# hirofumi0810/tensorflow_end2end_speech_recognition

Measured on AMD Instinct MI355X. Metric: acoustic frames/sec (train), TIMIT-shaped BLSTM-CTC, higher is better.
Workload: dtype bf16; 1 GPU; TIMIT 61-phone 5x256 BLSTM-CTC, B=16/GPU, D=120, C=62, seq_len~U{100..778}, dropout 0.2, rmsprop, train step; global_batch=16, parallelism=dp1, padded_to=own Tmax per rank

## Files before the change

### include/asr_hip.h

```cpp
#ifndef ASR_HIP_H_
#define ASR_HIP_H_

#include <stddef.h>
#include <stdint.h>

#ifdef __cplusplus
extern "C" {
#endif

typedef struct asr_handle asr_handle;
typedef void* asr_stream;

typedef enum {
  ASR_OK = 0,
  ASR_ERR_INVALID_ARG = -1,
  ASR_ERR_UNSUPPORTED = -2,
  ASR_ERR_HIP = -3,
  ASR_ERR_WORKSPACE = -4
} asr_status;

typedef enum { ASR_F32 = 0, ASR_BF16 = 1 } asr_dtype;

typedef enum {
  ASR_OPT_SGD = 0, ASR_OPT_MOMENTUM = 1, ASR_OPT_NESTEROV = 2, ASR_OPT_ADAGRAD = 3,
// ... 17 lines not shown
int asr_stack_frames(asr_handle* h, const float* x, const int32_t* seq_len, int B, int T, int F,
                     int num_stack, int num_skip, float* out, int32_t* out_len, asr_stream s);
int asr_splice(asr_handle* h, const float* x, const int32_t* seq_len, int B, int T, int D, int splice,
               int num_stack, float* out, asr_stream s);
int asr_transpose2d(asr_handle* h, int dtype, const void* in, int rows, int cols, int ld_in,
                    void* out, int ld_out, asr_stream s);
int asr_cast_from_f32(asr_handle* h, int dtype, const float* in, void* out, size_t n, asr_stream s);
int asr_cast_to_f32(asr_handle* h, int dtype, const void* in, float* out, size_t n, asr_stream s);
int asr_apply_mask(asr_handle* h, int dtype, const void* in, const float* mask, void* out,
                   size_t n, asr_stream s);
int asr_touch(asr_handle* h, const void* p, size_t bytes, asr_stream s);
int asr_dropout_mask(asr_handle* h, float* mask, size_t n, float keep_prob,
                     uint64_t seed, uint64_t offset, asr_stream s);
int asr_dropout_apply(asr_handle* h, int dtype, const void* in, void* out, size_t n, float keep_prob, uint64_t seed,
                      uint64_t offset, asr_stream s);
int asr_relu_bwd_drop(asr_handle* h, int dtype, const float* dout, const void* out, size_t n, float keep_prob,
                      uint64_t seed, uint64_t offset, void* dpre, asr_stream s);
int asr_colsum(asr_handle* h, int dtype, const void* a, int M, int N, int lda,
               float* out, asr_stream s);

int asr_gemm(asr_handle* h, int dtype, int out_dtype, int transA, int transB,
             int M, int N, int K, const void* A, int lda, const void* B, int ldb,
             void* C, int ldc, const float* bias, int accumulate, asr_stream s);

int asr_gemm_act(asr_handle* h, int dtype, int out_dtype, int transA, int transB,
                 int M, int N, int K, const void* A, int lda, const void* B, int ldb,
                 void* C, int ldc, const float* bias, int accumulate, int act, asr_stream s);
int asr_gemm_mul(asr_handle* h, int dtype, int transA, int transB, int M, int N, int K,
                 const void* A, int lda, const void* B, int ldb, float* C, int ldc,
                 const float* bias, int accumulate, int act, const float* mul, int ldmul, asr_stream s);
int asr_gemm_drop(asr_handle* h, int dtype, int transA, int transB, int M, int N, int K, const void* A, int lda,
                  const void* B, int ldb, float* C, int ldc, const float* bias, int accumulate, int act, float keep_prob,
                  uint64_t seed, uint64_t offset, asr_stream s);

int asr_im2col3x3(asr_handle* h, int dtype, const void* in, int N, int H, int W, int Cin, int ldp,
                  void* patches, asr_stream s);
int asr_col2im3x3(asr_handle* h, const float* dpatches, int N, int H, int W, int Cin, int ldp,
                  float* din, asr_stream s);
int asr_im2col(asr_handle* h, int dtype, const void* in_nhwc, int N, int H, int W, int Cin, int kh, int kw,
               int sh, int sw, int ldp, void* patches, asr_stream s);
int asr_col2im(asr_handle* h, const float* dpatches, int N, int H, int W, int Cin, int kh, int kw,
               int sh, int sw, int ldp, float* din_nhwc, asr_stream s);
int asr_conv3x3_prep_weights(asr_handle* h, const float* w_hwio, int Cin, int Cout, void* wt_fwd,
                             void* wt_bwd, asr_stream s);
int asr_conv3x3_fwd(asr_handle* h, const void* x, int N, int H, int W, int Cin, const void* wt_fwd,
                    const float* bias, int Cout, int relu, void* out, asr_stream s);
int asr_conv3x3_fwd_drop(asr_handle* h, const void* x, int N, int H, int W, int Cin, const void* wt_fwd,
                         const float* bias, int Cout, float keep_prob, uint64_t seed, uint64_t offset, void* out,
                         asr_stream s);
int asr_conv3x3_bwd_data(asr_handle* h, const void* dy, int N, int H, int W, int Cout,
                         const void* wt_bwd, int Cin, float* dx, asr_stream s);
int asr_conv3x3_bwd_data_relu(asr_handle* h, const void* dy, int N, int H, int W, int Cout, const void* wt_bwd, int Cin,
                              const void* act_below, float keep_prob, uint64_t seed, uint64_t offset, int use_drop,
                              void* dpre_below, asr_stream s);
int asr_conv3x3_bwd_weight(asr_handle* h, const void* x, const void* dy, int N, int H, int W,
                           int Cin, int Cout, float* dw, int accumulate, asr_stream s);
int asr_conv3x3_bwd_weight_bias(asr_handle* h, const void* x, const void* dy, int N, int H, int W,
                                int Cin, int Cout, float* dw, float* dbias, asr_stream s);
int asr_maxpool2x2_fwd(asr_handle* h, int dtype, const void* in, int N, int H, int W, int C,
                       void* out, uint8_t* argmax, asr_stream s);
int asr_maxpool2x2_fwd_drop(asr_handle* h, int dtype, const void* in, int N, int H, int W, int C, void* out,
                            uint8_t* argmax, float keep_prob, uint64_t seed, uint64_t offset, asr_stream s);
int asr_maxpool2x2_bwd(asr_handle* h, const float* dout, const uint8_t* argmax, int N, int H, int W,
                       int C, float* din, asr_stream s);
int asr_conv3x3_smallc_fwd(asr_handle* h, const void* x, int N, int H, int W, int Cin, const void* w2d,
                           const float* bias, int Cout, int relu, void* out, asr_stream s);
// ... 235 lines not shown
```

### tensorflow_end2end_speech_recognition_amd/_lib.py

```python
import ctypes as C
import os

_PKG = os.path.dirname(os.path.abspath(__file__))
LIB_PATH = os.path.join(_PKG, 'libasr_hip.so')

ASR_F32, ASR_BF16 = 0, 1
OPTIMIZER_IDS = {'sgd': 0, 'momentum': 1, 'nestrov': 2, 'adagrad': 3, 'adadelta': 4,
                 'rmsprop': 5, 'adam': 6}

_vp, _i, _f, _sz = C.c_void_p, C.c_int, C.c_float, C.c_size_t
_i64, _u64 = C.c_int64, C.c_uint64

SIGNATURES = {
    'asr_abi_version': (_i, []),
    'asr_create': (_i, [C.POINTER(_vp), _i]),
    'asr_create_ex': (_i, [C.POINTER(_vp), _i, _sz]),
    'asr_scratch_bytes': (_sz, [_vp]),
    'asr_destroy': (_i, [_vp]),
    'asr_set_xcd_skip': (_i, [_vp, _i]),
    'asr_set_gemm_tn_workgroups': (_i, [_vp, _i]),
    'asr_last_error_string': (C.c_char_p, [_vp]),
    'asr_device_info': (_i, [_vp, C.POINTER(_i), C.c_char_p, _i]),
    'asr_bt_to_tb': (_i, [_vp, _i, _vp, _vp, _i, _i, _i, _vp]),
    'asr_bt_to_tb_ld': (_i, [_vp, _i, _vp, _vp, _i, _i, _i, _i, _vp]),
    'asr_transpose2d': (_i, [_vp, _i, _vp, _i, _i, _i, _vp, _i, _vp]),
    'asr_cast_from_f32': (_i, [_vp, _i, _vp, _vp, _sz, _vp]),
    'asr_cast_to_f32': (_i, [_vp, _i, _vp, _vp, _sz, _vp]),
    'asr_apply_mask': (_i, [_vp, _i, _vp, _vp, _vp, _sz, _vp]),
    'asr_dropout_mask': (_i, [_vp, _vp, _sz, _f, _u64, _u64, _vp]),
    'asr_touch': (_i, [_vp, _vp, _sz, _vp]),
    'asr_dropout_apply': (_i, [_vp, _i, _vp, _vp, _sz, _f, _u64, _u64, _vp]),
    'asr_relu_bwd_drop': (_i, [_vp, _i, _vp, _vp, _sz, _f, _u64, _u64, _vp, _vp]),
    'asr_colsum': (_i, [_vp, _i, _vp, _i, _i, _i, _vp, _vp]),
    'asr_gemm': (_i, [_vp, _i, _i, _i, _i, _i, _i, _i, _vp, _i, _vp, _i, _vp, _i, _vp, _i, _vp]),
    'asr_gemm_act': (_i, [_vp, _i, _i, _i, _i, _i, _i, _i, _vp, _i, _vp, _i, _vp, _i, _vp, _i, _i, _vp]),
    'asr_gemm_drop': (_i, [_vp, _i, _i, _i, _i, _i, _i, _vp, _i, _vp, _i, _vp, _i, _vp, _i, _i, _f, _u64, _u64, _vp]),
    'asr_gemm_mul': (_i, [_vp, _i, _i, _i, _i, _i, _i, _vp, _i, _vp, _i, _vp, _i, _vp, _i, _i, _vp, _i, _vp]),
    'asr_conv3x3_prep_weights': (_i, [_vp, _vp, _i, _i, _vp, _vp, _vp]),
    'asr_conv3x3_fwd': (_i, [_vp, _vp, _i, _i, _i, _i, _vp, _vp, _i, _i, _vp, _vp]),
    'asr_conv3x3_fwd_drop': (_i, [_vp, _vp, _i, _i, _i, _i, _vp, _vp, _i, _f, _u64, _u64, _vp, _vp]),
    'asr_conv3x3_bwd_data': (_i, [_vp, _vp, _i, _i, _i, _i, _vp, _i, _vp, _vp]),
    'asr_conv3x3_smallc_fwd': (_i, [_vp, _vp, _i, _i, _i, _i, _vp, _vp, _i, _i, _vp, _vp]),
    'asr_conv3x3_smallc_fwd_drop': (_i, [_vp, _vp, _i, _i, _i, _i, _vp, _vp, _i, _f, _u64, _u64, _vp, _vp]),
    'asr_conv3x3_smallc_bwd_weight': (_i, [_vp, _vp, _vp, _i, _i, _i, _i, _i, _vp, _vp]),
    'asr_conv3x3_smallc_bwd_weight_bias': (_i, [_vp, _vp, _vp, _i, _i, _i, _i, _i, _vp, _vp, _vp]),
    'asr_conv3x3_bwd_data_relu': (_i, [_vp, _vp, _i, _i, _i, _i, _vp, _i, _vp, _f, _u64, _u64, _i, _vp, _vp]),
    'asr_conv3x3_bwd_weight': (_i, [_vp, _vp, _vp, _i, _i, _i, _i, _i, _vp, _i, _vp]),
    'asr_conv3x3_bwd_weight_bias': (_i, [_vp, _vp, _vp, _i, _i, _i, _i, _i, _vp, _vp, _vp]),
    'asr_im2col3x3': (_i, [_vp, _i, _vp, _i, _i, _i, _i, _i, _vp, _vp]),
    'asr_col2im3x3': (_i, [_vp, _vp, _i, _i, _i, _i, _i, _vp, _vp]),
    'asr_im2col': (_i, [_vp, _i, _vp, _i, _i, _i, _i, _i, _i, _i, _i, _i, _vp, _vp]),
    'asr_col2im': (_i, [_vp, _vp, _i, _i, _i, _i, _i, _i, _i, _i, _i, _vp, _vp]),
    'asr_maxpool2x2_fwd': (_i, [_vp, _i, _vp, _i, _i, _i, _i, _vp, _vp, _vp]),
    'asr_maxpool2x2_fwd_drop': (_i, [_vp, _i, _vp, _i, _i, _i, _i, _vp, _vp, _f, _u64, _u64, _vp]),
    'asr_relu_bwd_scaled': (_i, [_vp, _i, _vp, _vp, _sz, _f, _vp, _vp]),
    'asr_maxpool2x2_bwd': (_i, [_vp, _vp, _vp, _i, _i, _i, _i, _vp, _vp]),
    'asr_relu_bwd': (_i, [_vp, _i, _vp, _vp, _vp, _sz, _vp, _vp]),
    'asr_maxpool2x2_relu_bwd': (_i, [_vp, _i, _vp, _vp, _vp, _i, _i, _i, _i, _vp, _f, _u64, _u64, _i, _vp]),
    'asr_conv3x5_prep_weights': (_i, [_vp, _vp, _i, _i, _vp, _vp, _vp]),
    'asr_conv3x5_fwd': (_i, [_vp, _vp, _i, _i, _i, _i, _vp, _vp, _i, _i, _vp, _vp]),
    'asr_conv3x5_fwd_drop': (_i, [_vp, _vp, _i, _i, _i, _i, _vp, _vp, _i, _f, _u64, _u64, _vp, _vp]),
    'asr_conv3x5_bwd_data': (_i, [_vp, _vp, _i, _i, _i, _i, _vp, _i, _vp, _vp]),
    'asr_conv3x5_bwd_data_relu': (_i, [_vp, _vp, _i, _i, _i, _i, _vp, _i, _vp, _f, _u64, _u64, _i, _vp, _vp]),
    'asr_conv3x5_bwd_weight_bias': (_i, [_vp, _vp, _vp, _i, _i, _i, _i, _i, _vp, _vp, _vp]),
    'asr_maxpool3x1_fwd': (_i, [_vp, _i, _vp, _i, _i, _i, _i, _vp, _vp, _f, _u64, _u64, _i, _vp]),
    'asr_maxpool3x1_bwd': (_i, [_vp, _i, _vp, _vp, _i, _i, _i, _i, _vp, _vp]),
    'asr_lstm_prep_weights': (_i, [_vp, _i, _vp, _vp, _i, _i, _vp, _vp, _vp, _vp, _vp]),
    'asr_lstm_prep_layer': (_i, [_vp, _i, _i, _vp, _i, _i, _i, _vp, _vp, _vp, _vp, _vp, _vp, _vp]),
    'asr_lstm_grad_finish': (_i, [_vp, _i, _vp, _i, _i, _vp, _vp, _i, _vp]),
    'asr_gate_deinterleave': (_i, [_vp, _vp, _i, _vp, _i, _i, _i, _vp]),
# ... 147 lines not shown
```

### tensorflow_end2end_speech_recognition_amd/csrc/gemm.hip

```cpp
#include "common.h"
#include <stdlib.h>

namespace {

static inline bool first_on_device(unsigned long long& mask) {
  int d = 0;
  (void)hipGetDevice(&d);
  const unsigned long long bit = 1ull << (d & 63);
  if (mask & bit) return false;
  mask |= bit;
  return true;
}

template <typename T> struct GT;
template <> struct GT<float> {
  static constexpr int BK = 32;
  static constexpr int VEC = 4;
};
template <> struct GT<bf16_t> {
  static constexpr int BK = 64;
  static constexpr int VEC = 8;
};

template <typename T> struct Vec16 { T v[GT<T>::VEC]; } __attribute__((aligned(16)));
// ... 178 lines not shown
          *reinterpret_cast<f32x4_t*>(cp) = (f32x4_t){v[0], v[1], v[2], v[3]};
        } else {
          typedef __attribute__((ext_vector_type(4))) unsigned short us4_t;
          if (accumulate) {
            const us4_t o = *reinterpret_cast<const us4_t*>(cp);
#pragma unroll
            for (int r = 0; r < 4; ++r) v[r] += bf16_to_f32(o[r]);
          }
          if (act == 1) {
#pragma unroll
            for (int r = 0; r < 4; ++r) v[r] = fmaxf(v[r], 0.f);
          }
          *reinterpret_cast<us4_t*>(cp) = (us4_t){f32_to_bf16(v[0]), f32_to_bf16(v[1]), f32_to_bf16(v[2]), f32_to_bf16(v[3])};
        }
      } else {
        for (int r = 0; r < 4 && nb + r < N; ++r) {
          float w = v[r];
          if (accumulate) w += load_out<TO>(cp + r);
          if (act == 1) w = fmaxf(w, 0.f);
          store_out<TO>(cp + r, w);
        }
      }
    }
}

__device__ __forceinline__ unsigned nt_swz(int row) { return (((row + 4) >> 3) & 1) ? 8u : 0u; }

struct GemmDrop {
  float keep;
  uint64_t seed, offset;
  int use;
};

template <typename TO>
__global__ __launch_bounds__(256) void gemm_nt_bf16_kernel(int M, int N, int K, const bf16_t* __restrict__ A,
                                                           int lda, const bf16_t* __restrict__ Bt, int ldb,
                                                           TO* __restrict__ C, int ldc,
                                                           const float* __restrict__ bias, int accumulate,
                                                           int act, const float* __restrict__ mul, int ldm,
                                                           GemmDrop drop) {
  constexpr int BM = 128, BN = 128, BK = 64, LD = BK + 8;
  constexpr int STAGE = (BM + BN) * LD;
  extern __shared__ __attribute__((aligned(16))) char smem[];
  bf16_t* S = reinterpret_cast<bf16_t*>(smem);

  const int tid = threadIdx.x, lane = tid & 63, wave = tid >> 6;
  const int wm = wave >> 1, wn = wave & 1;
  const int ntn = N / BN, ntm = (M + BM - 1) / BM, total = ntn * ntm;
  int t = blockIdx.x;
  if ((total & 7) == 0) t = (t & 7) * (total >> 3) + (t >> 3);
  const int m0 = (t / ntn) * BM, n0 = (t % ntn) * BN;

  const bf16_t* pa[4];
  const bf16_t* pb[4];
  unsigned so[4];
#pragma unroll
  for (int i = 0; i < 4; ++i) {
    const int v = tid + i * 256, r = v >> 3, kv = (v & 7) * 8;
    pa[i] = A + (size_t)min(m0 + r, M - 1) * lda + kv;
    pb[i] = Bt + (size_t)(n0 + r) * ldb + kv;
    so[i] = (unsigned)(r * LD) + ((unsigned)kv ^ nt_swz(r));
  }
  bf16x8_t ra[4], rb[4];
  auto gload = [&]() {
#pragma unroll
    for (int i = 0; i < 4; ++i) {
      ra[i] = *reinterpret_cast<const bf16x8_t*>(pa[i]);
      rb[i] = *reinterpret_cast<const bf16x8_t*>(pb[i]);
      pa[i] += BK;
      pb[i] += BK;
    }
  };
  auto sstore = [&](bf16_t* st) {
#pragma unroll
    for (int i = 0; i < 4; ++i) {
      *reinterpret_cast<bf16x8_t*>(st + so[i]) = ra[i];
      *reinterpret_cast<bf16x8_t*>(st + BM * LD + so[i]) = rb[i];
    }
  };

  f32x4_t acc[4][4];
#pragma unroll
  for (int i = 0; i < 4; ++i)
#pragma unroll
    for (int j = 0; j < 4; ++j) acc[i][j] = (f32x4_t){0.f, 0.f, 0.f, 0.f};

  const int nkt = K / BK;
  gload();
  sstore(S);
  __syncthreads();
  const int fr = lane & 15, fq = lane >> 4;
  const unsigned aoff = (unsigned)((wm * 64 + fr) * LD) + ((unsigned)(fq * 8) ^ nt_swz(fr));
  const unsigned boff = (unsigned)(BM * LD + (wn * 64 + fr) * LD) + ((unsigned)(fq * 8) ^ nt_swz(fr));
  for (int kt = 0; kt < nkt; ++kt) {
    const bf16_t* cur = S + (kt & 1) * STAGE;
    if (kt + 1 < nkt) gload();
#pragma unroll
    for (int ks = 0; ks < 2; ++ks) {
      bf16x8_t a[4], b[4];
#pragma unroll
      for (int i = 0; i < 4; ++i) a[i] = *reinterpret_cast<const bf16x8_t*>(cur + aoff + i * 16 * LD + ks * 32);
#pragma unroll
      for (int j = 0; j < 4; ++j) b[j] = *reinterpret_cast<const bf16x8_t*>(cur + boff + j * 16 * LD + ks * 32);
#pragma unroll
      for (int i = 0; i < 4; ++i)
#pragma unroll
        for (int j = 0; j < 4; ++j)
          acc[i][j] = __builtin_amdgcn_mfma_f32_16x16x32_bf16(b[j], a[i], acc[i][j], 0, 0, 0);
    }
    if (kt + 1 < nkt) sstore(S + ((kt + 1) & 1) * STAGE);
    __syncthreads();
  }
#pragma unroll
  for (int i = 0; i < 4; ++i) {
    const int m = m0 + wm * 64 + i * 16 + fr;
    if (m >= M) continue;
#pragma unroll
    for (int j = 0; j < 4; ++j) {
      const int nb = n0 + wn * 64 + j * 16 + fq * 4;
      TO* cp = C + (size_t)m * ldc + nb;
      float v[4];
#pragma unroll
      for (int r = 0; r < 4; ++r) v[r] = acc[i][j][r];
      if (bias) {
        const f32x4_t bv = *reinterpret_cast<const f32x4_t*>(bias + nb);
#pragma unroll
        for (int r = 0; r < 4; ++r) v[r] += bv[r];
      }
      if constexpr (sizeof(TO) == 4) {
        if (accumulate) {
          const f32x4_t o = *reinterpret_cast<const f32x4_t*>(cp);
#pragma unroll
          for (int r = 0; r < 4; ++r) v[r] += o[r];
        }
        if (act == 1) {
#pragma unroll
          for (int r = 0; r < 4; ++r) v[r] = fmaxf(v[r], 0.f);
        }
        if (mul) {
          const f32x4_t mv = *reinterpret_cast<const f32x4_t*>(mul + (size_t)m * ldm + nb);
#pragma unroll
          for (int r = 0; r < 4; ++r) v[r] *= mv[r];
        }
        if (drop.use) {
          float mk[4];
          asr_dropout_words(drop.offset + ((size_t)m * N + nb) / 4, drop.seed, drop.keep, 1.f / drop.keep, mk);
#pragma unroll
          for (int r = 0; r < 4; ++r) v[r] *= mk[r];
        }
        *reinterpret_cast<f32x4_t*>(cp) = (f32x4_t){v[0], v[1], v[2], v[3]};
      } else {
        typedef __attribute__((ext_vector_type(4))) unsigned short us4_t;
        if (accumulate) {
          const us4_t o = *reinterpret_cast<const us4_t*>(cp);
#pragma unroll
          for (int r = 0; r < 4; ++r) v[r] += bf16_to_f32(o[r]);
// ... 136 lines not shown
        if (accumulate) {
          const us4_t o = *reinterpret_cast<const us4_t*>(cp);
#pragma unroll
          for (int r = 0; r < 4; ++r) v[r] += bf16_to_f32(o[r]);
        }
        if (act == 1) {
#pragma unroll
          for (int r = 0; r < 4; ++r) v[r] = fmaxf(v[r], 0.f);
        }
        *reinterpret_cast<us4_t*>(cp) = (us4_t){f32_to_bf16(v[0]), f32_to_bf16(v[1]), f32_to_bf16(v[2]), f32_to_bf16(v[3])};
      }
    }
  }
}

template <typename TO, int BM, int BN, int WM, int WN>
static void launch_gemm_nt_big(int M, int N, int K, const void* A, int lda, const void* B, int ldb, void* C, int ldc,
                               const float* bias, int accumulate, hipStream_t st, int act, const float* mul, int ldm,
                               GemmDrop drop) {
  const size_t lds = (size_t)2 * (BM + BN) * (64 + 8) * sizeof(bf16_t);
  static unsigned long long attr_done = 0;
  auto k = gemm_nt_bf16_big_kernel<TO, BM, BN, WM, WN>;
  if (first_on_device(attr_done)) {
    (void)hipFuncSetAttribute((const void*)k, hipFuncAttributeMaxDynamicSharedMemorySize, (int)lds);
  }
  const long tiles = (long)(N / BN) * ((M + BM - 1) / BM);
  hipLaunchKernelGGL(k, dim3((unsigned)tiles), dim3(WM * WN * 64), lds, st, M, N, K, (const bf16_t*)A, lda,
                     (const bf16_t*)B, ldb, (TO*)C, ldc, bias, accumulate, act, mul, ldm, drop);
}

template <typename TO>
bool try_gemm_nt_bf16(int transA, int transB, int M, int N, int K, const void* A, int lda, const void* B,
                      int ldb, void* C, int ldc, const float* bias, int accumulate, hipStream_t st, int act,
                      const float* mul, int ldm, GemmDrop drop = GemmDrop{1.f, 0, 0, 0}) {
  if (transA || !transB || K % 64 != 0 || N % 128 != 0 || M < 1024) return false;
  if (drop.use && sizeof(TO) != 4) return false;
  if (mul && (sizeof(TO) != 4 || ldm % 4 != 0 || ((uintptr_t)mul) % 16 != 0)) return false;
  if (lda % 8 != 0 || ldb % 8 != 0 || ((uintptr_t)A) % 16 != 0 || ((uintptr_t)B) % 16 != 0) return false;
  if (ldc % 4 != 0 || ((uintptr_t)C) % (4 * sizeof(TO)) != 0 || (bias && ((uintptr_t)bias) % 16 != 0)) return false;
  static const int big = [] { const char* e = getenv("ASR_GEMM_NT_BIG"); return e ? atoi(e) : 1; }();
  const bool fits32 = ((size_t)(M - 1) * lda + K) * sizeof(bf16_t) < 0xFFFFFFFFull && ((size_t)(N - 1) * ldb + K) * sizeof(bf16_t) < 0xFFFFFFFFull;
  const long tiles256 = (long)(N / 256) * ((M + 255) / 256);
  if (big && fits32 && N % 256 == 0 && (big == 2 ? M >= 2048 : tiles256 >= 512)) {
    launch_gemm_nt_big<TO, 256, 256, 2, 4>(M, N, K, A, lda, B, ldb, C, ldc, bias, accumulate, st, act, mul, ldm, drop);
    return true;
  }
  const size_t lds = (size_t)2 * (128 + 128) * (64 + 8) * sizeof(bf16_t);
  static unsigned long long attr_done = 0;
  if (first_on_device(attr_done)) {
    (void)hipFuncSetAttribute((const void*)gemm_nt_bf16_kernel<TO>, hipFuncAttributeMaxDynamicSharedMemorySize, (int)lds);
  }
  const int total = (N / 128) * ((M + 127) / 128);
  hipLaunchKernelGGL(gemm_nt_bf16_kernel<TO>, dim3(total), dim3(256), lds, st, M, N, K, (const bf16_t*)A, lda,
                     (const bf16_t*)B, ldb, (TO*)C, ldc, bias, accumulate, act, mul, ldm, drop);
  return true;
}

__device__ __forceinline__ int xcd_work_index(int skip) {
  const int b = blockIdx.x, x = b & 7;
  if (x < skip) return -1;
  return (b >> 3) * (8 - skip) + (x - skip);
}
static inline unsigned xcd_grid(long work, int skip) {
  const long per = 8 - skip;
  return (unsigned)((work + per - 1) / per * 8);
}

constexpr int SK_WAVES = 8;
struct SkinnyCell {
  const float *c_prev, *h_prev, *peep, *live, *out_mask;
  float *gates, *c_raw, *c_out, *h_out, *h_raw, *cell_out, *h_out2, *cell_out2;
  int U, ld_h2, ld_c2;
  float fb, clip;
};
__device__ __forceinline__ float sk_sigf(float x) { return 1.0f / (1.0f + expf(-x)); }
template <bool TRANSB, int NT, bool CELL = false, bool BH = false>
__global__ __launch_bounds__(64 * SK_WAVES) void gemm_skinny_f32_kernel(int M, int N, int K, const float* __restrict__ A,
                                                                        int lda, const float* __restrict__ Bm, int ldb,
                                                                        float* __restrict__ C, int ldc,
                                                                        const float* __restrict__ bias, int accumulate,
// ... 948 lines not shown
#pragma unroll
      for (int u = 0; u < 8; ++u) t[u] = partial[(size_t)(z + u) * total + i];
#pragma unroll
      for (int u = 0; u < 8; ++u) v += t[u];
    }
    for (; z < S; ++z) v += partial[(size_t)z * total + i];
    TO* cp = C + (size_t)m * ldc + n;
    if (accumulate) v += load_out<TO>(cp);
    if (act == 1) v = fmaxf(v, 0.f);
    store_out<TO>(cp, v);
  }
}

template <typename T, typename TO, int BM, int BN>
int launch_layout(int transA, int transB, dim3 grid, size_t lds, hipStream_t st, int M, int N, int K,
                  const T* A, int lda, const T* B, int ldb, TO* C, int ldc, const float* bias,
                  int accumulate, int aa, int ba, int kchunk, float* partial, int act) {
  const int c_vec = (((uintptr_t)C) % (4 * sizeof(TO)) == 0) && (ldc % 4 == 0);
#define ASR_GEMM_LAUNCH(TA_, TB_)                                                             \
  hipLaunchKernelGGL((gemm_kernel<T, TO, BM, BN, TA_, TB_>), grid, dim3(256), lds, st, M, N, K, A, \
                     lda, B, ldb, C, ldc, bias, accumulate, aa, ba, kchunk, partial, act, c_vec)
  if (!transA && !transB) ASR_GEMM_LAUNCH(false, false);
  else if (!transA && transB) ASR_GEMM_LAUNCH(false, true);
  else if (transA && !transB) ASR_GEMM_LAUNCH(true, false);
  else ASR_GEMM_LAUNCH(true, true);
#undef ASR_GEMM_LAUNCH
  return 0;
}

template <typename T, typename TO>
int launch_gemm(asr_handle* h, int transA, int transB, int M, int N, int K, const void* A, int lda,
                const void* B, int ldb, void* C, int ldc, const float* bias, int accumulate,
                hipStream_t st, int act, const float* mul = nullptr, int ldm = 0, bool* mul_done = nullptr,
                GemmDrop drop = GemmDrop{1.f, 0, 0, 0}) {
  constexpr int VEC = GT<T>::VEC, BK = GT<T>::BK;
  if constexpr (sizeof(T) == 4 && sizeof(TO) == 4) {
    if (try_gemm_skinny_f32(transA, transB, M, N, K, A, lda, B, ldb, C, ldc, bias, accumulate, st, act)) return 0;
  }
  if constexpr (sizeof(T) == 2) {
    if (try_gemm_nt_bf16<TO>(transA, transB, M, N, K, A, lda, B, ldb, C, ldc, bias, accumulate, st, act, mul, ldm, drop)) {
      if (mul_done) *mul_done = true;
      return 0;
    }
    if (transA && !transB && K >= 2048 && M % 8 == 0 && N % 8 == 0 && lda % 8 == 0 && ldb % 8 == 0 &&
        ((uintptr_t)A) % 16 == 0 && ((uintptr_t)B) % 16 == 0) {
      const int tm = (M + 127) / 128, tn = (N + 127) / 128;
      const int tn_wgs = h->tn_wgs > 0 ? h->tn_wgs : 512;
      int S = (tn_wgs + tm * tn - 1) / (tm * tn);
      const int maxS = (K + 255) / 256;
      if (S > maxS) S = maxS;
      if (S > 256) S = 256;
      while (S > 1 && (size_t)S * M * N * sizeof(float) > h->scratch_bytes - ASR_XCH_BYTES) --S;
      if ((size_t)S * M * N * sizeof(float) <= h->scratch_bytes - ASR_XCH_BYTES) {
        int kchunk = (K + S - 1) / S;
        kchunk = (kchunk + 63) / 64 * 64;
        S = (K + kchunk - 1) / kchunk;
        const size_t lds = (size_t)2 * TN_STAGE;
        static unsigned long long attr_done = 0;
        if (first_on_device(attr_done)) {
          (void)hipFuncSetAttribute((const void*)gemm_tn_bf16_kernel, hipFuncAttributeMaxDynamicSharedMemorySize, (int)lds);
        }
        float* partial = (float*)h->scratch;
        const int skip = h->xcd_skip;
        hipLaunchKernelGGL(gemm_tn_bf16_kernel, dim3(xcd_grid((long)tn * tm * S, skip)), dim3(256), lds, st, M, N, K,
                           (const bf16_t*)A, lda, (const bf16_t*)B, ldb, kchunk, partial, tn, tm, S, skip);
        const size_t total = (size_t)M * N;
        int blocks = (int)((total + 255) / 256);
        if (blocks > 2048) blocks = 2048;
        hipLaunchKernelGGL(splitk_reduce_kernel<TO>, dim3(xcd_grid(blocks, skip)), dim3(256), 0, st, partial, S, M, N,
                           (TO*)C, ldc, bias, accumulate, act, skip);
        return 0;
      }
    }
// ... 133 lines not shown
    launch_gemm<float, float>(h, transA, transB, M, N, K, A, lda, B, ldb, C, ldc, bias, accumulate, st, act, mul, ldmul, &fused);
  else
    launch_gemm<bf16_t, float>(h, transA, transB, M, N, K, A, lda, B, ldb, C, ldc, bias, accumulate, st, act, mul, ldmul, &fused);
  ASR_CHECK_LAUNCH(h, "asr_gemm_mul");
  if (!fused) {
    const size_t total = (size_t)M * N;
    int blocks = (int)((total + 255) / 256);
    if (blocks > 2048) blocks = 2048;
    hipLaunchKernelGGL(mul_rows_kernel, dim3(blocks), dim3(256), 0, st, C, ldc, mul, ldmul, M, N);
    ASR_CHECK_LAUNCH(h, "asr_gemm_mul(multiply)");
  }
  return ASR_OK;
}

extern "C" int asr_dropout_apply(asr_handle* h, int dtype, const void* in, void* out, size_t n, float keep_prob,
                                 uint64_t seed, uint64_t offset, asr_stream s);
extern "C" int asr_gemm_drop(asr_handle* h, int dtype, int transA, int transB, int M, int N, int K, const void* A,
                             int lda, const void* B, int ldb, float* C, int ldc, const float* bias, int accumulate,
                             int act, float keep_prob, uint64_t seed, uint64_t offset, asr_stream s) {
  if (!h) return ASR_ERR_INVALID_ARG;
  if (!asr_dtype_ok(dtype) || (act != 0 && act != 1) || M < 0 || N < 0 || K < 0 || !A || !B || !C ||
      lda < (transA ? M : K) || ldb < (transB ? K : N) || ldc != N || N % 4 != 0 || !(keep_prob > 0.f && keep_prob <= 1.f))
    ASR_FAIL(h, ASR_ERR_INVALID_ARG, "asr_gemm_drop: bad args M=%d N=%d K=%d ldc=%d (ldc == N, N %% 4 == 0)", M, N, K, ldc);
  if (M == 0 || N == 0) return ASR_OK;
  hipStream_t st = (hipStream_t)s;
  bool fused = false;
  const GemmDrop drop = {keep_prob, seed, offset, 1};
  if (dtype == ASR_F32)
    launch_gemm<float, float>(h, transA, transB, M, N, K, A, lda, B, ldb, C, ldc, bias, accumulate, st, act, nullptr, 0, &fused, drop);
  else
    launch_gemm<bf16_t, float>(h, transA, transB, M, N, K, A, lda, B, ldb, C, ldc, bias, accumulate, st, act, nullptr, 0, &fused, drop);
  ASR_CHECK_LAUNCH(h, "asr_gemm_drop");
  if (!fused) return asr_dropout_apply(h, ASR_F32, C, C, (size_t)M * N, keep_prob, seed, offset, s);
  return ASR_OK;
}

extern "C" int asr_conv3x3_prep_weights(asr_handle* h, const float* w_hwio, int Cin, int Cout, void* wt_fwd,
                                        void* wt_bwd, asr_stream s) {
  if (!h) return ASR_ERR_INVALID_ARG;
  if (!w_hwio || !wt_fwd || !wt_bwd || Cin < 1 || Cout < 1)
    ASR_FAIL(h, ASR_ERR_INVALID_ARG, "asr_conv3x3_prep_weights: bad args");
  const size_t total = (size_t)9 * Cin * Cout;
  int blocks = (int)((total + 255) / 256);
  if (blocks > 1024) blocks = 1024;
  hipLaunchKernelGGL(conv3x3_prep_kernel, dim3(blocks), dim3(256), 0, (hipStream_t)s, w_hwio, Cin, Cout,
                     (bf16_t*)wt_fwd, (bf16_t*)wt_bwd);
  ASR_CHECK_LAUNCH(h, "asr_conv3x3_prep_weights");
  return ASR_OK;
}

static unsigned long long* g_convdbg_host = nullptr;
extern "C" int asr_debug_conv_cycles(unsigned long long* out, int n) {
  if (!g_convdbg_host || n > 64 * 4 * 8) return -1;
  return hipMemcpy(out, g_convdbg_host, n * sizeof(unsigned long long), hipMemcpyDeviceToHost) == hipSuccess ? 0 : -3;
}
template <typename TO>
static int conv3x3_launch(asr_handle* h, const void* x, int Nimg, int H, int W, int Cin, const void* wt,
                          const float* bias, int Cout, int act, void* out, hipStream_t st,
                          ConvGate gate = ConvGate{nullptr, 1.f, 0, 0, 0}) {
  const long long mp = (long long)Nimg * H * W;
  if (mp <= 0 || mp >= (1ll << 31)) ASR_FAIL(h, ASR_ERR_UNSUPPORTED, "asr_conv3x3: %lld pixels", mp);
  const int Mpix = (int)mp;
  {
    static const bool img_on = [] { const char* e = getenv("ASR_CONV_IMG"); return !(e && e[0] == '0'); }();
    const size_t img_bytes = (size_t)(H + 2) * (W + 2) * (Cin * 2 + 16);
    const int nvec = H * W * Cin / 8;
// ... 506 lines not shown
```

### tensorflow_end2end_speech_recognition_amd/models/encoders/core/rnn_util.py

```python
import os as _os

import numpy as np
import torch

from .... import ops
from ...._lib import ASR_BF16, ASR_F32

DIRS = ('fw', 'bw')
DW_LANES = 2
FORK_ONCE = _os.environ.get('ASR_FORK_ONCE', '1') != '0'
BG_WGS = int(_os.environ.get('ASR_BG_WGS', '128'))
DW_AFTER_DX_FLOPS = {'0': float('inf'), '1': 0.0}.get(_os.environ.get('ASR_DW_AFTER_DX', ''), 2e11)


def declare_lstm_vars(store, scope, din, H, ndir, use_peephole, parameter_init, rng, cell_scope=None):
    names = []
    for d in range(ndir):
        base = '%s/%s/lstm_cell' % (scope, DIRS[d]) if cell_scope is None else cell_scope
        u = lambda *s: rng.uniform(-parameter_init, parameter_init, size=s)
        store.declare(base + '/kernel', (din + H, 4 * H), u(din + H, 4 * H))
        store.declare(base + '/bias', (4 * H,), np.zeros(4 * H))
        if use_peephole:
            store.declare(base + '/w_i_diag', (H,), u(H))
            store.declare(base + '/w_f_diag', (H,), u(H))
# ... 18 lines not shown
        rows = []
        for b in self.bases:
            row = [view(b + '/kernel'), view(b + '/bias')]
            row += [view(b + '/w_i_diag'), view(b + '/w_f_diag'), view(b + '/w_o_diag')] if self.use_peephole \
                else [None, None, None]
            rows.append(tuple(row))
        return rows

    def prepare(self, device, dtype, T, B, keep_prob=1.0, is_training=True, rng_state=None, drop_mask=None,
                ldk=None):
        w = ops.lstm_prep_layer(self._vars(self.store.__getitem__), self.din, self.H, dtype, ldk=ldk)
        w['mask'] = self.make_mask(device, T, B, keep_prob, is_training, rng_state, drop_mask)
        return w

    def make_mask(self, device, T, B, keep_prob=1.0, is_training=True, rng_state=None, drop_mask=None):
        if not (is_training and (drop_mask is not None or keep_prob < 1.0)):
            return None
        if drop_mask is not None:
            return drop_mask
        seed, offset = rng_state
        return (float(keep_prob), int(seed), int(offset))

    @staticmethod
    def _masked(t, mask):
        return ops.dropout_apply(t, *mask) if isinstance(mask, tuple) else ops.apply_mask(t, mask)

    def forward(self, x, seq_len, dtype, keep_prob=1.0, is_training=True, rng_state=None,
                drop_mask=None, save=True, prep=None, mask_event=None):
        T, B, ldk = x.shape
        H, ndir = self.H, self.ndir
        if prep is None:
            prep = self.prepare(x.device, dtype, T, B, keep_prob, is_training, rng_state, drop_mask, ldk=ldk)
        xproj = torch.empty((T, B, ndir * 4 * H), dtype=torch.float32, device=x.device)
        ops.gemm(x.view(T * B, ldk), prep['wxT'], transB=True, bias=prep['bias'],
                 out=xproj.view(T * B, ndir * 4 * H))
        gates, hout, cs, cf, hf = ops.lstm_fwd(xproj, prep['whf'], prep['peep'], seq_len, H, ndir, dtype,
                                               self.forget_bias, self.cell_clip or 0.0)
        out = hout
        mask = prep['mask']
        if mask is not None:
            if not isinstance(mask, tuple):
                ops.wait_event(mask_event)
            out = self._masked(hout, mask)
        if save:
            self.ctx = dict(x=x, gates=gates, cs=cs, hout=hout, whb=prep['whb'], peep=prep['peep'],
                            seq_len=seq_len, dtype=dtype, mask=mask, wx_cat=prep['wx_cat'])
        return out, (cf, hf)

    def backward(self, dout, d_c_final=None, d_h_final=None, need_dx=True, dout_masked=False, dx_mask=None,
                 background=False, warm=None, acc=None, finish=True):
        c = self.ctx
        st = self.store
        dtype = c['dtype']
        x, hout = c['x'], c['hout']
        T, B, ldk = x.shape
        din, H, ndir = self.din, self.H, self.ndir
        if c['mask'] is not None and not dout_masked:
            dout = self._masked(dout, c['mask'])
        dgates, dpeep = ops.lstm_bwd(dout, c['gates'], c['cs'], c['whb'], c['peep'], c['seq_len'], H,
                                     ndir, dtype, d_c_final, d_h_final, want_dpeep=True)
        self.warm_event = None
        fork = ops.stream_event() if FORK_ONCE else None
        if warm:
            with ops.side_lane(dout.device, keep=tuple(warm), lane=2, after=fork):
                for t in warm:
                    ops.touch(t)
                if not FORK_ONCE:
                    self.warm_event = ops.stream_event()
        x2d = x.view(T * B, ldk)[:, :din]
        h2d = hout.view(T * B, ndir * H)
        dg2d = dgates.view(T * B, ndir * 4 * H)
        dx = torch.empty((T, B, din), dtype=torch.float32, device=x.device) if need_dx else None
        if need_dx:
            if isinstance(dx_mask, tuple):
                ops.gemm(dg2d, c['wx_cat'], transB=True, out=dx.view(T * B, din), drop=dx_mask)
            else:
                ops.gemm(dg2d, c['wx_cat'], transB=True, out=dx.view(T * B, din),
                         mul=dx_mask.view(T * B, din) if dx_mask is not None else None)
            if FORK_ONCE and background and 2.0 * T * B * din * ndir * 4 * H >= DW_AFTER_DX_FLOPS:
                fork = ops.stream_event()
        add = acc is not None
        dw_il = acc['dw_il'] if add else \
            torch.empty((ndir, din + H, 4 * H), dtype=torch.float32, device=x.device)
        ops.set_side_gemm_workgroups(x.device, BG_WGS if background else 0)
        done = []
        for d in range(ndir):
            with ops.side_lane(x.device, keep=(x, hout, dgates, dpeep, dw_il), lane=1 + (d % DW_LANES), after=fork):
                dg = dg2d[:, d * 4 * H:(d + 1) * 4 * H]
                ops.gemm(x2d, dg, transA=True, out=dw_il[d, :din], accumulate=add)
                if T > 1:
                    if d == 0:
                        ops.gemm(h2d[:(T - 1) * B, d * H:(d + 1) * H], dg[B:], transA=True, out=dw_il[d, din:],
                                 accumulate=add)
                    else:
                        ops.gemm(h2d[B:, d * H:(d + 1) * H], dg[:(T - 1) * B], transA=True, out=dw_il[d, din:],
                                 accumulate=add)
                elif not add:
                    dw_il[d, din:].zero_()
                if d % DW_LANES > 0:
                    done.append(ops.stream_event())
        if not finish:
            self.acc = dict(dw_il=dw_il, dpeep=dpeep)
            self.ctx = None
            return dx
        with ops.side_lane(x.device, keep=(dpeep,), lane=1, after=fork):
            for ev in done:
                ops.wait_event(ev)
            if add:
                dpeep = acc['dpeep'] + dpeep
                ops.keep_on_lane(x.device, 1, (dpeep,))
            ops.lstm_grad_finish(self._vars(st.g), dw_il, dpeep, H)
# ... 297 lines not shown
```

### tensorflow_end2end_speech_recognition_amd/ops.py

```python
import ctypes as C
import os
import time as _time

import numpy as np
import torch

from . import _lib
from ._lib import ASR_BF16, ASR_F32

TORCH_DTYPE = {ASR_F32: torch.float32, ASR_BF16: torch.bfloat16}


def dtype_id(dtype):
    if dtype in (ASR_F32, 'f32', 'fp32', 'float32', torch.float32):
        return ASR_F32
    if dtype in (ASR_BF16, 'bf16', 'bfloat16', torch.bfloat16):
        return ASR_BF16
    raise ValueError('dtype must be f32 or bf16, got %r' % (dtype,))


_lane = 0
_side = {}


# ... 334 lines not shown
    odt = dt if out_dtype is None else dtype_id(out_dtype)
    if out is None:
        out = torch.empty((M, N), dtype=TORCH_DTYPE[odt], device=A.device)
    else:
        odt = dtype_id(out.dtype)
        if out.shape != (M, N) or out.stride(1) != 1:
            raise ValueError('gemm: bad out shape %s' % (tuple(out.shape),))
    if bias is not None:
        _chk(bias, torch.float32, 'bias')
    if drop is not None:
        if odt != ASR_F32 or not out.is_contiguous() or N % 4:
            raise ValueError('gemm: drop needs a contiguous fp32 output with N % 4 == 0')
        h.check(h.lib.asr_gemm_drop(h.h, dt, int(transA), int(transB), M, N, K,
                                    C.c_void_p(A.data_ptr()), A.stride(0), C.c_void_p(B.data_ptr()), B.stride(0),
                                    C.c_void_p(out.data_ptr()), out.stride(0), _p(bias), int(accumulate),
                                    1 if relu else 0, float(drop[0]), int(drop[1]), int(drop[2]), _s()), 'asr_gemm_drop')
        return out
    if mul is not None:
        _chk(mul, torch.float32, 'mul')
        if odt != ASR_F32 or mul.dim() != 2 or mul.shape != (M, N) or mul.stride(1) != 1:
            raise ValueError('gemm: mul needs an fp32 output and an fp32 [M,N] multiplier')
        h.check(h.lib.asr_gemm_mul(h.h, dt, int(transA), int(transB), M, N, K,
                                   C.c_void_p(A.data_ptr()), A.stride(0), C.c_void_p(B.data_ptr()), B.stride(0),
                                   C.c_void_p(out.data_ptr()), out.stride(0), _p(bias), int(accumulate),
                                   1 if relu else 0, C.c_void_p(mul.data_ptr()), mul.stride(0), _s()), 'asr_gemm_mul')
        return out
    h.check(h.lib.asr_gemm_act(h.h, dt, odt, int(transA), int(transB), M, N, K,
                               C.c_void_p(A.data_ptr()), A.stride(0), C.c_void_p(B.data_ptr()), B.stride(0),
                               C.c_void_p(out.data_ptr()), out.stride(0), _p(bias), int(accumulate),
                               1 if relu else 0, _s()), 'asr_gemm')
    return out


def conv3x3_prep_weights(w_hwio):
    h = _h(w_hwio)
    _chk(w_hwio, torch.float32, 'w')
    _, _, Cin, Cout = w_hwio.shape
    wf = torch.empty((Cout, 9 * Cin), dtype=torch.bfloat16, device=w_hwio.device)
    wb = torch.empty((Cin, 9 * Cout), dtype=torch.bfloat16, device=w_hwio.device)
    h.check(h.lib.asr_conv3x3_prep_weights(h.h, _p(w_hwio.contiguous()), Cin, Cout, _p(wf), _p(wb), _s()),
            'asr_conv3x3_prep_weights')
    return wf, wb


def _out_like(out, shape, dtype, device, what):
    if out is None:
        return torch.empty(shape, dtype=dtype, device=device)
    if tuple(out.shape) != tuple(shape) or out.dtype != dtype or not out.is_contiguous():
        raise ValueError('%s: out must be a contiguous %s tensor of shape %s' % (what, dtype, tuple(shape)))
    return out


def conv3x3_fwd(x_nhwc, wt_fwd, bias, relu=True, out=None):
    h = _h(x_nhwc)
    _chk(x_nhwc, torch.bfloat16, 'x')
    N, H, W, Cin = x_nhwc.shape
    Cout = wt_fwd.shape[0]
    out = _out_like(out, (N, H, W, Cout), torch.bfloat16, x_nhwc.device, 'conv3x3_fwd')
    h.check(h.lib.asr_conv3x3_fwd(h.h, _p(x_nhwc), N, H, W, Cin, _p(wt_fwd), _p(bias), Cout, 1 if relu else 0,
                                  _p(out), _s()), 'asr_conv3x3_fwd')
    return out


def conv3x3_fwd_drop(x_nhwc, wt_fwd, bias, drop, out=None):
    h = _h(x_nhwc)
    _chk(x_nhwc, torch.bfloat16, 'x')
# ... 1140 lines not shown
```

Before: 723,700 frames/s.

## Skip padded frames in LSTM input and dx GEMMs via ragged tile scheduling

Adds a ragged variant of the bf16 NT GEMM kernel that reads per-utterance sequence lengths on device and launches tiles only over valid frames of each utterance, remapping rows from time-major layout. The LSTM input projection and the backward dx GEMM now use it, so work on padding frames past each utterance's length is skipped. In fill mode, tiles that are entirely padding are zeroed without any K loop. The cost is extra in-kernel prefix-sum work for scheduling, strided row gathers across the batch that may hurt A-tile memory coalescing, and smaller effective M per tile.

```diff
diff --git a/include/asr_hip.h b/include/asr_hip.h
--- a/include/asr_hip.h
+++ b/include/asr_hip.h
@@ -73,6 +73,9 @@
 int asr_gemm_drop(asr_handle* h, int dtype, int transA, int transB, int M, int N, int K, const void* A, int lda,
                   const void* B, int ldb, float* C, int ldc, const float* bias, int accumulate, int act, float keep_prob,
                   uint64_t seed, uint64_t offset, asr_stream s);
+int asr_gemm_ragged(asr_handle* h, int M, int N, int K, const void* A, int lda, const void* B, int ldb, float* C, int ldc,
+                    const float* bias, int accumulate, int act, const float* mul, int ldmul, int use_drop, float keep_prob,
+                    uint64_t seed, uint64_t offset, const int* seq_len, int Bu, int fill, asr_stream s);
 
 int asr_im2col3x3(asr_handle* h, int dtype, const void* in, int N, int H, int W, int Cin, int ldp,
                   void* patches, asr_stream s);
diff --git a/tensorflow_end2end_speech_recognition_amd/_lib.py b/tensorflow_end2end_speech_recognition_amd/_lib.py
--- a/tensorflow_end2end_speech_recognition_amd/_lib.py
+++ b/tensorflow_end2end_speech_recognition_amd/_lib.py
@@ -36,6 +36,8 @@
     'asr_gemm_act': (_i, [_vp, _i, _i, _i, _i, _i, _i, _i, _vp, _i, _vp, _i, _vp, _i, _vp, _i, _i, _vp]),
     'asr_gemm_drop': (_i, [_vp, _i, _i, _i, _i, _i, _i, _vp, _i, _vp, _i, _vp, _i, _vp, _i, _i, _f, _u64, _u64, _vp]),
     'asr_gemm_mul': (_i, [_vp, _i, _i, _i, _i, _i, _i, _vp, _i, _vp, _i, _vp, _i, _vp, _i, _i, _vp, _i, _vp]),
+    'asr_gemm_ragged': (_i, [_vp, _i, _i, _i, _vp, _i, _vp, _i, _vp, _i, _vp, _i, _i, _vp, _i, _i, _f, _u64, _u64, _vp, _i,
+                             _i, _vp]),
     'asr_conv3x3_prep_weights': (_i, [_vp, _vp, _i, _i, _vp, _vp, _vp]),
     'asr_conv3x3_fwd': (_i, [_vp, _vp, _i, _i, _i, _i, _vp, _vp, _i, _i, _vp, _vp]),
     'asr_conv3x3_fwd_drop': (_i, [_vp, _vp, _i, _i, _i, _i, _vp, _vp, _i, _f, _u64, _u64, _vp, _vp]),
diff --git a/tensorflow_end2end_speech_recognition_amd/csrc/gemm.hip b/tensorflow_end2end_speech_recognition_amd/csrc/gemm.hip
--- a/tensorflow_end2end_speech_recognition_amd/csrc/gemm.hip
+++ b/tensorflow_end2end_speech_recognition_amd/csrc/gemm.hip
@@ -234,13 +234,18 @@
   int use;
 };
 
-template <typename TO>
+struct GemmRagged {
+  const int* seq_len;
+  int Bu, fill;
+};
+
+template <typename TO, bool RAG = false>
 __global__ __launch_bounds__(256) void gemm_nt_bf16_kernel(int M, int N, int K, const bf16_t* __restrict__ A,
                                                            int lda, const bf16_t* __restrict__ Bt, int ldb,
                                                            TO* __restrict__ C, int ldc,
                                                            const float* __restrict__ bias, int accumulate,
                                                            int act, const float* __restrict__ mul, int ldm,
-                                                           GemmDrop drop) {
+                                                           GemmDrop drop, GemmRagged rag = GemmRagged{nullptr, 1, 0}) {
   constexpr int BM = 128, BN = 128, BK = 64, LD = BK + 8;
   constexpr int STAGE = (BM + BN) * LD;
   extern __shared__ __attribute__((aligned(16))) char smem[];
@@ -248,10 +253,54 @@
 
   const int tid = threadIdx.x, lane = tid & 63, wave = tid >> 6;
   const int wm = wave >> 1, wn = wave & 1;
-  const int ntn = N / BN, ntm = (M + BM - 1) / BM, total = ntn * ntm;
-  int t = blockIdx.x;
-  if ((total & 7) == 0) t = (t & 7) * (total >> 3) + (t >> 3);
-  const int m0 = (t / ntn) * BM, n0 = (t % ntn) * BN;
+  const int ntn = N / BN;
+  int m0, n0;
+  int ub = 0, len = 0;
+  bool dead = false;
+  if constexpr (!RAG) {
+    const int ntm = (M + BM - 1) / BM, total = ntn * ntm;
+    int t = blockIdx.x;
+    if ((total & 7) == 0) t = (t & 7) * (total >> 3) + (t >> 3);
+    m0 = (t / ntn) * BM;
+    n0 = (t % ntn) * BN;
+  } else {
+    const int Bu = rag.Bu, T = M / Bu, ntb = (T + BM - 1) / BM;
+    const int l = lane < Bu ? min(max(rag.seq_len[lane], 0), T) : 0;
+    const int c = (l + BM - 1) / BM;
+    int inc = c;
+#pragma unroll
+    for (int o = 1; o < 64; o <<= 1) {
+      const int y = __shfl_up(inc, o);
+      if (lane >= o) inc += y;
+    }
+    const int live = __shfl(inc, 63), total = live * ntn;
+    int t = blockIdx.x, mt, cnt, exc;
+    if (t < total) {
+      if ((total & 7) == 0) t = (t & 7) * (total >> 3) + (t >> 3);
+      mt = t / ntn;
+      cnt = inc;
+      exc = inc - c;
+    } else {
+      if (!rag.fill) return;
+      t -= total;
+      mt = t / ntn;
+      const int dc = lane < Bu ? ntb - c : 0;
+      int dinc = dc;
+#pragma unroll
+      for (int o = 1; o < 64; o <<= 1) {
+        const int y = __shfl_up(dinc, o);
+        if (lane >= o) dinc += y;
+      }
+      if (mt >= __shfl(dinc, 63)) return;
+      cnt = dinc;
+      exc = dinc - dc - c;
+      dead = true;
+    }
+    ub = __popcll(__ballot(lane < Bu && cnt <= mt));
+    m0 = (mt - __shfl(exc, ub)) * BM;
+    len = __shfl(l, ub);
+    n0 = (t % ntn) * BN;
+  }
 
   const bf16_t* pa[4];
   const bf16_t* pb[4];
@@ -259,7 +308,10 @@
 #pragma unroll
   for (int i = 0; i < 4; ++i) {
     const int v = tid + i * 256, r = v >> 3, kv = (v & 7) * 8;
-    pa[i] = A + (size_t)min(m0 + r, M - 1) * lda + kv;
+    if constexpr (RAG)
+      pa[i] = A + ((size_t)max(min(m0 + r, len - 1), 0) * rag.Bu + ub) * lda + kv;
+    else
+      pa[i] = A + (size_t)min(m0 + r, M - 1) * lda + kv;
     pb[i] = Bt + (size_t)(n0 + r) * ldb + kv;
     so[i] = (unsigned)(r * LD) + ((unsigned)kv ^ nt_swz(r));
   }
@@ -287,9 +339,11 @@
 #pragma unroll
     for (int j = 0; j < 4; ++j) acc[i][j] = (f32x4_t){0.f, 0.f, 0.f, 0.f};
 
-  const int nkt = K / BK;
-  gload();
-  sstore(S);
+  const int nkt = dead ? 0 : K / BK;
+  if (!dead) {
+    gload();
+    sstore(S);
+  }
   __syncthreads();
   const int fr = lane & 15, fq = lane >> 4;
   const unsigned aoff = (unsigned)((wm * 64 + fr) * LD) + ((unsigned)(fq * 8) ^ nt_swz(fr));
@@ -315,15 +369,23 @@
   }
 #pragma unroll
   for (int i = 0; i < 4; ++i) {
-    const int m = m0 + wm * 64 + i * 16 + fr;
-    if (m >= M) continue;
+    int m = m0 + wm * 64 + i * 16 + fr;
+    bool pad = false;
+    if constexpr (RAG) {
+      const int tt = m;
+      if (tt >= M / rag.Bu || (tt >= len && !rag.fill)) continue;
+      pad = tt >= len;
+      m = tt * rag.Bu + ub;
+    } else {
+      if (m >= M) continue;
+    }
 #pragma unroll
     for (int j = 0; j < 4; ++j) {
       const int nb = n0 + wn * 64 + j * 16 + fq * 4;
       TO* cp = C + (size_t)m * ldc + nb;
       float v[4];
 #pragma unroll
-      for (int r = 0; r < 4; ++r) v[r] = acc[i][j][r];
+      for (int r = 0; r < 4; ++r) v[r] = pad ? 0.f : acc[i][j][r];
       if (bias) {
         const f32x4_t bv = *reinterpret_cast<const f32x4_t*>(bias + nb);
 #pragma unroll
@@ -526,7 +588,8 @@
 template <typename TO>
 bool try_gemm_nt_bf16(int transA, int transB, int M, int N, int K, const void* A, int lda, const void* B,
                       int ldb, void* C, int ldc, const float* bias, int accumulate, hipStream_t st, int act,
-                      const float* mul, int ldm, GemmDrop drop = GemmDrop{1.f, 0, 0, 0}) {
+                      const float* mul, int ldm, GemmDrop drop = GemmDrop{1.f, 0, 0, 0},
+                      GemmRagged rag = GemmRagged{nullptr, 1, 0}) {
   if (transA || !transB || K % 64 != 0 || N % 128 != 0 || M < 1024) return false;
   if (drop.use && sizeof(TO) != 4) return false;
   if (mul && (sizeof(TO) != 4 || ldm % 4 != 0 || ((uintptr_t)mul) % 16 != 0)) return false;
@@ -540,6 +603,19 @@
     return true;
   }
   const size_t lds = (size_t)2 * (128 + 128) * (64 + 8) * sizeof(bf16_t);
+  static const bool rag_on = [] { const char* e = getenv("ASR_GEMM_RAGGED"); return !(e && e[0] == '0'); }();
+  if (rag.seq_len && rag_on && rag.Bu >= 1 && rag.Bu <= 64 && M % rag.Bu == 0 &&
+      (size_t)rag.Bu * lda <= 0x7FFFFFFFu) {
+    static unsigned long long rag_attr = 0;
+    if (first_on_device(rag_attr)) {
+      (void)hipFuncSetAttribute((const void*)gemm_nt_bf16_kernel<TO, true>, hipFuncAttributeMaxDynamicSharedMemorySize,
+                                (int)lds);
+    }
+    const long grid = (long)rag.Bu * ((M / rag.Bu + 127) / 128) * (N / 128);
+    hipLaunchKernelGGL((gemm_nt_bf16_kernel<TO, true>), dim3((unsigned)grid), dim3(256), lds, st, M, N, K, (const bf16_t*)A,
+                       lda, (const bf16_t*)B, ldb, (TO*)C, ldc, bias, accumulate, act, mul, ldm, drop, rag);
+    return true;
+  }
   static unsigned long long attr_done = 0;
   if (first_on_device(attr_done)) {
     (void)hipFuncSetAttribute((const void*)gemm_nt_bf16_kernel<TO>, hipFuncAttributeMaxDynamicSharedMemorySize, (int)lds);
@@ -1554,13 +1630,14 @@
 int launch_gemm(asr_handle* h, int transA, int transB, int M, int N, int K, const void* A, int lda,
                 const void* B, int ldb, void* C, int ldc, const float* bias, int accumulate,
                 hipStream_t st, int act, const float* mul = nullptr, int ldm = 0, bool* mul_done = nullptr,
-                GemmDrop drop = GemmDrop{1.f, 0, 0, 0}) {
+                GemmDrop drop = GemmDrop{1.f, 0, 0, 0}, GemmRagged rag = GemmRagged{nullptr, 1, 0}) {
   constexpr int VEC = GT<T>::VEC, BK = GT<T>::BK;
   if constexpr (sizeof(T) == 4 && sizeof(TO) == 4) {
     if (try_gemm_skinny_f32(transA, transB, M, N, K, A, lda, B, ldb, C, ldc, bias, accumulate, st, act)) return 0;
   }
   if constexpr (sizeof(T) == 2) {
-    if (try_gemm_nt_bf16<TO>(transA, transB, M, N, K, A, lda, B, ldb, C, ldc, bias, accumulate, st, act, mul, ldm, drop)) {
+    if (try_gemm_nt_bf16<TO>(transA, transB, M, N, K, A, lda, B, ldb, C, ldc, bias, accumulate, st, act, mul, ldm, drop,
+                             rag)) {
       if (mul_done) *mul_done = true;
       return 0;
     }
@@ -1760,6 +1837,35 @@
     launch_gemm<bf16_t, float>(h, transA, transB, M, N, K, A, lda, B, ldb, C, ldc, bias, accumulate, st, act, nullptr, 0, &fused, drop);
   ASR_CHECK_LAUNCH(h, "asr_gemm_drop");
   if (!fused) return asr_dropout_apply(h, ASR_F32, C, C, (size_t)M * N, keep_prob, seed, offset, s);
+  return ASR_OK;
+}
+
+extern "C" int asr_gemm_ragged(asr_handle* h, int M, int N, int K, const void* A, int lda, const void* B, int ldb, float* C,
+                               int ldc, const float* bias, int accumulate, int act, const float* mul, int ldmul,
+                               int use_drop, float keep_prob, uint64_t seed, uint64_t offset, const int* seq_len, int Bu,
+                               int fill, asr_stream s) {
+  if (!h) return ASR_ERR_INVALID_ARG;
+  if ((act != 0 && act != 1) || M < 0 || N < 0 || K < 0 || !A || !B || !C || !seq_len || Bu < 1 || M % Bu != 0 ||
+      lda < K || ldb < K || ldc < N || (mul && ldmul < N) || (mul && use_drop) || (fill != 0 && fill != 1) ||
+      (use_drop && (ldc != N || N % 4 != 0 || !(keep_prob > 0.f && keep_prob <= 1.f))))
+    ASR_FAIL(h, ASR_ERR_INVALID_ARG, "asr_gemm_ragged: bad args M=%d N=%d K=%d lda=%d ldb=%d ldc=%d Bu=%d", M, N, K, lda,
+             ldb, ldc, Bu);
+  if (M == 0 || N == 0) return ASR_OK;
+  hipStream_t st = (hipStream_t)s;
+  bool fused = false;
+  const GemmDrop drop = {keep_prob, seed, offset, use_drop ? 1 : 0};
+  const GemmRagged rag = {seq_len, Bu, fill};
+  launch_gemm<bf16_t, float>(h, 0, 1, M, N, K, A, lda, B, ldb, C, ldc, bias, accumulate, st, act, mul, mul ? ldmul : 0,
+                             &fused, drop, rag);
+  ASR_CHECK_LAUNCH(h, "asr_gemm_ragged");
+  if (!fused && use_drop) return asr_dropout_apply(h, ASR_F32, C, C, (size_t)M * N, keep_prob, seed, offset, s);
+  if (!fused && mul) {
+    const size_t total = (size_t)M * N;
+    int blocks = (int)((total + 255) / 256);
+    if (blocks > 2048) blocks = 2048;
+    hipLaunchKernelGGL(mul_rows_kernel, dim3(blocks), dim3(256), 0, st, C, ldc, mul, ldmul, M, N);
+    ASR_CHECK_LAUNCH(h, "asr_gemm_ragged(multiply)");
+  }
   return ASR_OK;
 }
 
diff --git a/tensorflow_end2end_speech_recognition_amd/models/encoders/core/rnn_util.py b/tensorflow_end2end_speech_recognition_amd/models/encoders/core/rnn_util.py
--- a/tensorflow_end2end_speech_recognition_amd/models/encoders/core/rnn_util.py
+++ b/tensorflow_end2end_speech_recognition_amd/models/encoders/core/rnn_util.py
@@ -74,8 +74,7 @@
         if prep is None:
             prep = self.prepare(x.device, dtype, T, B, keep_prob, is_training, rng_state, drop_mask, ldk=ldk)
         xproj = torch.empty((T, B, ndir * 4 * H), dtype=torch.float32, device=x.device)
-        ops.gemm(x.view(T * B, ldk), prep['wxT'], transB=True, bias=prep['bias'],
-                 out=xproj.view(T * B, ndir * 4 * H))
+        ops.gemm_frames(x.view(T * B, ldk), prep['wxT'], seq_len, bias=prep['bias'], out=xproj.view(T * B, ndir * 4 * H))
         gates, hout, cs, cf, hf = ops.lstm_fwd(xproj, prep['whf'], prep['peep'], seq_len, H, ndir, dtype,
                                                self.forget_bias, self.cell_clip or 0.0)
         out = hout
@@ -115,10 +114,10 @@
         dx = torch.empty((T, B, din), dtype=torch.float32, device=x.device) if need_dx else None
         if need_dx:
             if isinstance(dx_mask, tuple):
-                ops.gemm(dg2d, c['wx_cat'], transB=True, out=dx.view(T * B, din), drop=dx_mask)
+                ops.gemm_frames(dg2d, c['wx_cat'], c['seq_len'], out=dx.view(T * B, din), drop=dx_mask, fill=True)
             else:
-                ops.gemm(dg2d, c['wx_cat'], transB=True, out=dx.view(T * B, din),
-                         mul=dx_mask.view(T * B, din) if dx_mask is not None else None)
+                ops.gemm_frames(dg2d, c['wx_cat'], c['seq_len'], out=dx.view(T * B, din),
+                                mul=dx_mask.view(T * B, din) if dx_mask is not None else None, fill=True)
             if FORK_ONCE and background and 2.0 * T * B * din * ndir * 4 * H >= DW_AFTER_DX_FLOPS:
                 fork = ops.stream_event()
         add = acc is not None
diff --git a/tensorflow_end2end_speech_recognition_amd/ops.py b/tensorflow_end2end_speech_recognition_amd/ops.py
--- a/tensorflow_end2end_speech_recognition_amd/ops.py
+++ b/tensorflow_end2end_speech_recognition_amd/ops.py
@@ -390,6 +390,39 @@
     return out
 
 
+def gemm_frames(A, B, seq_len, bias=None, out=None, mul=None, drop=None, fill=False):
+    if A.dtype != torch.bfloat16 or A.device.type != 'cuda' or (out is not None and out.dtype != torch.float32):
+        return gemm(A, B, transB=True, bias=bias, out=out, out_dtype=torch.float32, mul=mul, drop=drop)
+    h = _h(A)
+    _chk(seq_len, torch.int32, 'seq_len')
+    if B.dtype != A.dtype or A.dim() != 2 or B.dim() != 2 or A.stride(1) != 1 or B.stride(1) != 1:
+        raise ValueError('gemm: ragged product needs 2-D bf16 operands with unit inner stride')
+    M, K = A.shape
+    N = B.shape[0]
+    Bu = seq_len.numel()
+    if B.shape[1] != K or M % Bu:
+        raise ValueError('gemm: ragged product: bad shapes A %s B %s, %d utterances' % (tuple(A.shape), tuple(B.shape), Bu))
+    if out is None:
+        out = torch.empty((M, N), dtype=torch.float32, device=A.device)
+    elif out.shape != (M, N) or out.stride(1) != 1:
+        raise ValueError('gemm: bad out shape %s' % (tuple(out.shape),))
+    if bias is not None:
+        _chk(bias, torch.float32, 'bias')
+    if mul is not None:
+        _chk(mul, torch.float32, 'mul')
+        if mul.dim() != 2 or mul.shape != (M, N) or mul.stride(1) != 1:
+            raise ValueError('gemm: mul needs an fp32 [M,N] multiplier')
+    if drop is not None and (not out.is_contiguous() or N % 4):
+        raise ValueError('gemm: drop needs a contiguous fp32 output with N % 4 == 0')
+    kp, seed, off = drop if drop is not None else (1.0, 0, 0)
+    h.check(h.lib.asr_gemm_ragged(h.h, M, N, K, C.c_void_p(A.data_ptr()), A.stride(0), C.c_void_p(B.data_ptr()),
+                                  B.stride(0), C.c_void_p(out.data_ptr()), out.stride(0), _p(bias), 0, 0, C.c_void_p(mul.data_ptr()) if mul is not None else None,
+                                  mul.stride(0) if mul is not None else 0,
+                                  1 if drop is not None else 0, float(kp), int(seed), int(off), _p(seq_len), Bu,
+                                  1 if fill else 0, _s()), 'asr_gemm_ragged')
+    return out
+
+
 def conv3x3_prep_weights(w_hwio):
     h = _h(w_hwio)
     _chk(w_hwio, torch.float32, 'w')
```

Measured after the change: 728,500 frames/s, median of 6. Within noise of the previous version (+0.7%).
